# joesound212985/Deepfake-Detection-using-CLIP-Based-SigLIP-2-Vision-Transformers

Measured on AMD Instinct MI355X. Metric: images/sec (train fwd+bwd) SigLIP-2-so400m@384 bf16, higher is better.
Workload: dtype bf16; 1 GPU; so400m-patch14-384 encoder+pool-head train fwd+bwd, 384x384, per-GPU batch 128, seeded random weights; global_batch=128, parallelism=dp1

## Files before the change

deepfake-detection-using-clip-based-siglip-2-vision-transformers_amd/csrc/attention.hip:

```cpp
#include <stdlib.h>

#include "common.hip.h"
#include "kernels.h"

namespace sgl {

hipError_t attn_f32_fwd(const float*, const float*, const float*, float*, float*, int, int, int, int, int, int, hipStream_t);
hipError_t attn_f32_bwd(const float*, const float*, const float*, const float*, const float*, const float*, float*,
                        float*, int, int, int, int, int, int, hipStream_t);
hipError_t attn_ref_fwd(const float*, const float*, const float*, float*, float*, int, int, int, int, int, int, hipStream_t);
hipError_t attn_ref_bwd(const float*, const float*, const float*, const float*, const float*, const float*, float*,
                        float*, int, int, int, int, int, int, hipStream_t);

template <int DP>
struct AttnCfg {
  static constexpr int KS = DP / 16;
  static constexpr int DT = (DP + 31) / 32;
  static constexpr int CPR = DP / 8;
  static constexpr int RSTR = DP * 2 + 16;
  static constexpr int TSTR = 192;
  static constexpr int DSTR = 208;
};

__device__ __forceinline__ u32x4 a_ldg(__amdgpu_buffer_rsrc_t r, uint32_t off) {
  return __builtin_amdgcn_raw_buffer_load_b128(r, off, 0, 0);
}
template <typename T>
__device__ __forceinline__ lo_x8<T> as_x8(u32x4 v) { return __builtin_bit_cast(lo_x8<T>, v); }
template <typename T>
__device__ __forceinline__ lo_x8<T> lds_row8(const char* p) { return *reinterpret_cast<const lo_x8<T>*>(p); }
template <typename T>
__device__ __forceinline__ lo_x4<T> lds_tr4(const char* p) { return lds_read_tr16<T>(p); }
template <typename T>
__device__ __forceinline__ lo_x8<T> lds_trfrag(const char* img, int stride, int kk, int dcol0, int lane) {
  const int g = lane >> 4, q = (lane >> 2) & 3, p = lane & 3;
  const char* a = img + (16 * kk + 4 * (g >> 1) + q) * stride + (dcol0 + 16 * (g & 1) + 4 * p) * 2;
  const lo_x4<T> lo = lds_tr4<T>(a);
  const lo_x4<T> hi = lds_tr4<T>(a + 8 * stride);
  return __builtin_shufflevector(lo, hi, 0, 1, 2, 3, 4, 5, 6, 7);
}
template <typename T>
__device__ __forceinline__ lo_x8<T> pack8(const f32x16& s, int base) {
  lo_x8<T> r;
#pragma unroll
  for (int j = 0; j < 8; ++j) r[j] = (T)s[base + j];
  return r;
}
__device__ __forceinline__ float fast_exp2(float x) { return __builtin_amdgcn_exp2f(x); }

__device__ __forceinline__ bool head_block(int nb, int BH, int& bh, int& xb) {
  const int pid = blockIdx.x, xcd = pid & 7, slot = pid >> 3;
  const int hq = slot / nb;
  bh = hq * 8 + xcd;
  xb = slot - hq * nb;
  return bh < BH;
}
static inline dim3 head_grid(int nb, int BH) { return dim3((unsigned)(8 * ((BH + 7) / 8) * nb)); }

struct HeadSrc {
  uint32_t rowbytes, nc, bytes;
  size_t base;
};
__device__ __forceinline__ HeadSrc head_src(int ld, int b, int hd, int H, int N, int dh, int DP) {
  HeadSrc r;
  if (ld > 0) {
    r.rowbytes = (uint32_t)ld * 2u;
    r.nc = (uint32_t)dh / 8u;
    r.bytes = (uint32_t)(((size_t)(N - 1) * ld + dh) * 2);
    r.base = (size_t)b * N * ld + (size_t)hd * dh;
  } else {
    r.rowbytes = (uint32_t)DP * 2u;
    r.nc = (uint32_t)DP / 8u;
    r.bytes = (uint32_t)((size_t)N * DP * 2);
    r.base = ((size_t)b * H + hd) * (size_t)N * DP;
  }
  return r;
}

#define MFMA32(a, b, c) mfma_32x32x16((a), (b), (c))

__device__ __forceinline__ void att_dma16(u32x4 desc, uint32_t lds_addr, uint32_t voff) {
  asm volatile("s_mov_b32 m0, %0\n\ts_nop 0\n\tbuffer_load_dwordx4 %1, %2, 0 offen lds" ::"s"(lds_addr), "v"(voff), "s"(desc)
               : "memory");
}
__device__ __forceinline__ void att_dma4(u32x4 desc, uint32_t lds_addr, uint32_t voff) {
  asm volatile("s_mov_b32 m0, %0\n\ts_nop 0\n\tbuffer_load_dword %1, %2, 0 offen lds" ::"s"(lds_addr), "v"(voff), "s"(desc)
               : "memory");
}
__device__ __forceinline__ u32x4 att_desc(const void* base, uint32_t bytes) {
  const uint64_t q = (uint64_t)base;
  return u32x4{(uint32_t)q, (uint32_t)(q >> 32) & 0xffffu, bytes, 0x00020000u};
}
__device__ __forceinline__ uint32_t att_chunk_off(int cidx, int rows, int SC, int NC, uint32_t rowbytes) {
  const int row = cidx / SC, col = cidx - row * SC;
  return (row < rows && col < NC) ? (uint32_t)row * rowbytes + (uint32_t)col * 16u : SGL_OOB;
}
#define SGL_ATT_WAIT_BARRIER(n)                                   \
  do {                                                            \
    asm volatile("s_waitcnt vmcnt(" #n ") lgkmcnt(0)" ::: "memory"); \
    __builtin_amdgcn_sched_barrier(0);                            \
    __builtin_amdgcn_s_barrier();                                 \
    __builtin_amdgcn_sched_barrier(0);                            \
    asm volatile("" ::: "memory");                                \
  } while (0)

template <typename T, int DP, bool TOK>
__global__ __launch_bounds__(256) __attribute__((amdgpu_waves_per_eu(3, 3))) void attn_fwd_kernel(const T* __restrict__ Q, const T* __restrict__ K,
                                                          const T* __restrict__ V, T* __restrict__ out,
                                                          float* __restrict__ lse, int B, int H, int N, int dh, int ld,
                                                          float c, float scale) {
  using C = AttnCfg<DP>;
  constexpr int KT = 64;
  constexpr int KBYTES = KT * C::RSTR, VBYTES = KT * C::TSTR, STAGE = KBYTES + VBYTES;
  constexpr int SCK = C::RSTR / 16, SCV = C::TSTR / 16;
  constexpr int NIK = KT * SCK / 64, NIV = KT * SCV / 64, NSLOT = NIK + NIV;
  constexpr int NPW = (NSLOT + 3) / 4;
  static_assert(KT * SCK % 64 == 0 && KT * SCV % 64 == 0, "whole DMA instructions per image");
  extern __shared__ __attribute__((aligned(16))) char smem[];
  const int t = threadIdx.x, lane = t & 63;
  const int w = __builtin_amdgcn_readfirstlane(t >> 6);
  int bh, xb;
  if (!head_block((N + 127) / 128, B * H, bh, xb)) return;
  const int b = bh / H, hd = bh - b * H;
  const int q0 = xb * 128 + w * 32;
  HeadSrc src = head_src(TOK ? ld : 0, b, hd, H, N, dh, DP);
  if constexpr (!TOK) {
    src.rowbytes = (uint32_t)DP * 2u;
    src.nc = (uint32_t)DP / 8u;
  }
  const __amdgpu_buffer_rsrc_t rq = make_rsrc(Q + src.base, src.bytes);
  const u32x4 dk_ = att_desc(K + src.base, src.bytes);
  const u32x4 dv_ = att_desc(V + src.base, src.bytes);
  const uint32_t lds0 = (uint32_t)(size_t)((SGL_LDS char*)smem);

  const int qi = lane & 31, hh = lane >> 5;
  lo_x8<T> qf[C::KS];
#pragma unroll
  for (int ks = 0; ks < C::KS; ++ks) {
    const uint32_t ch = (uint32_t)(2 * ks + hh);
    qf[ks] = as_x8<T>(a_ldg(rq, (q0 + qi < N && ch < src.nc) ? (uint32_t)(q0 + qi) * src.rowbytes + ch * 16u : SGL_OOB));
  }

  uint32_t voff[NPW];
#pragma unroll
  for (int j = 0; j < NPW; ++j) {
    const int sl = w + 4 * j;
    voff[j] = (sl < NIK) ? att_chunk_off(sl * 64 + lane, KT, SCK, (int)src.nc, src.rowbytes)
                         : att_chunk_off((sl - NIK) * 64 + lane, KT, SCV, (int)src.nc, src.rowbytes);
  }
  const uint32_t tile_adv = (uint32_t)KT * src.rowbytes;
  auto issue = [&](int stage) {
    const uint32_t sb = lds0 + (uint32_t)(stage * STAGE);
#pragma unroll
    for (int j = 0; j < NPW; ++j) {
      const int sl = w + 4 * j;
      if (sl < NSLOT) att_dma16(sl < NIK ? dk_ : dv_, sb + (uint32_t)sl * 1024u, voff[j]);
      voff[j] += tile_adv;
    }
  };

  float m_run = -INFINITY, l_run = 0.f;
  f32x16 o[C::DT];
#pragma unroll
  for (int dt = 0; dt < C::DT; ++dt)
#pragma unroll
    for (int r = 0; r < 16; ++r) o[dt][r] = 0.f;

  const int ntiles = (N + KT - 1) / KT;
#pragma unroll
  for (int ks = 0; ks < C::KS; ++ks) asm volatile("" ::"v"(qf[ks]));
  asm volatile("s_waitcnt vmcnt(0)" ::: "memory");
  issue(0);
  for (int tile = 0; tile < ntiles; ++tile) {
    const int cur = tile & 1;
    SGL_ATT_WAIT_BARRIER(0);
    if (tile + 1 < ntiles) issue(cur ^ 1);
    const char* kb = smem + cur * STAGE;
    const char* vb = kb + KBYTES;
    f32x16 s0, s1;
#pragma unroll
    for (int r = 0; r < 16; ++r) { s0[r] = 0.f; s1[r] = 0.f; }
#pragma unroll
    for (int ks = 0; ks < C::KS; ++ks) {
      const lo_x8<T> k0 = lds_row8<T>(kb + qi * C::RSTR + (16 * ks + 8 * hh) * 2);
      const lo_x8<T> k1 = lds_row8<T>(kb + (qi + 32) * C::RSTR + (16 * ks + 8 * hh) * 2);
      s0 = MFMA32(k0, qf[ks], s0);
      s1 = MFMA32(k1, qf[ks], s1);
    }
    if (tile == ntiles - 1) {
#pragma unroll
      for (int r = 0; r < 16; ++r) {
        const int key = tile * KT + (r & 3) + 8 * (r >> 2) + 4 * hh;
        if (key >= N) s0[r] = -INFINITY;
        if (key + 32 >= N) s1[r] = -INFINITY;
      }
    }
    float mx = s0[0];
#pragma unroll
    for (int r = 1; r < 16; ++r) mx = fmaxf(mx, s0[r]);
#pragma unroll
    for (int r = 0; r < 16; ++r) mx = fmaxf(mx, s1[r]);
    mx = fmaxf(mx, __shfl_xor(mx, 32, 64));
    const float m_new = fmaxf(m_run, mx);
    const bool grew = __any(m_new > m_run);
    const float alpha = grew ? fast_exp2(c * (m_run - m_new)) : 1.0f;
    const float mc = m_new * c;
    float rs = 0.f;
#pragma unroll
    for (int r = 0; r < 16; ++r) {
      s0[r] = fast_exp2(fmaf(s0[r], c, -mc));
      s1[r] = fast_exp2(fmaf(s1[r], c, -mc));
      rs += s0[r] + s1[r];
    }
    l_run = l_run * alpha + rs;
    m_run = m_new;
    if (grew) {
#pragma unroll
      for (int dt = 0; dt < C::DT; ++dt)
#pragma unroll
        for (int r = 0; r < 16; ++r) o[dt][r] *= alpha;
    }
    lo_x8<T> pb[4];
    pb[0] = pack8<T>(s0, 0);
    pb[1] = pack8<T>(s0, 8);
    pb[2] = pack8<T>(s1, 0);
    pb[3] = pack8<T>(s1, 8);
#pragma unroll
    for (int dt = 0; dt < C::DT; ++dt)
#pragma unroll
      for (int kk = 0; kk < 4; ++kk) o[dt] = MFMA32(lds_trfrag<T>(vb, C::TSTR, kk, dt * 32, lane), pb[kk], o[dt]);
  }
  const float l = l_run + __shfl_xor(l_run, 32, 64);
  const float inv = 1.0f / l;
  const int q = q0 + qi;
  if (q < N) {
    T* orow = out + ((size_t)b * N + q) * ((size_t)H * dh) + hd * dh;
#pragma unroll
    for (int dt = 0; dt < C::DT; ++dt)
#pragma unroll
      for (int g4 = 0; g4 < 4; ++g4) {
        const int d = dt * 32 + 8 * g4 + 4 * hh;
        if (d < dh) {
          lo_x4<T> v4;
#pragma unroll
          for (int r = 0; r < 4; ++r) v4[r] = (T)(o[dt][4 * g4 + r] * inv);
          *reinterpret_cast<lo_x4<T>*>(orow + d) = v4;
        }
      }
    if (hh == 0) lse[(size_t)bh * N + q] = m_run * scale + __logf(l);
  }
}

template <typename T, int DP, bool TOK>
__global__ __launch_bounds__(256, 2) void attn_bwd_kv_kernel(const T* __restrict__ Q, const T* __restrict__ K,
                                                             const T* __restrict__ V, const T* __restrict__ dO,
                                                             const float* __restrict__ aux, T* __restrict__ dqkv,
                                                             int B, int H, int N, int dh, int ld, float c, float scale) {
  using C = AttnCfg<DP>;
  constexpr int QT = 32;
  constexpr int SC = C::DSTR / 16;
  constexpr int NIS = (QT * SC + 63) / 64;
  constexpr int IMG = NIS * 1024;
  constexpr int STAGE = 2 * IMG + QT * 8;
  constexpr int NSLOT = 2 * NIS + 1;
  static_assert(NSLOT <= 16 && NSLOT > 12, "four DMA slots per wave (three for the last wave)");
  extern __shared__ __attribute__((aligned(16))) char smem[];
  const int t = threadIdx.x, lane = t & 63;
  const int w = __builtin_amdgcn_readfirstlane(t >> 6);
  int bh, xb;
  if (!head_block((N + 127) / 128, B * H, bh, xb)) return;
  const int b = bh / H, hd = bh - b * H;
  const int D = H * dh;
  const int key0 = xb * 128 + w * 32;
  HeadSrc src = head_src(TOK ? ld : 0, b, hd, H, N, dh, DP);
  if constexpr (!TOK) {
    src.rowbytes = (uint32_t)DP * 2u;
    src.nc = (uint32_t)DP / 8u;
  }
  const __amdgpu_buffer_rsrc_t rk = make_rsrc(K + src.base, src.bytes);
  const __amdgpu_buffer_rsrc_t rv = make_rsrc(V + src.base, src.bytes);
  const T* dOb = dO + (size_t)b * N * D + hd * dh;
  const u32x4 dq_ = att_desc(Q + src.base, src.bytes);
  const u32x4 ddo = att_desc(dOb, (uint32_t)(((size_t)(N - 1) * D + dh) * 2));
  const u32x4 dax = att_desc(aux + (size_t)bh * N * 2, (uint32_t)((size_t)N * 8));
  const uint32_t lds0 = (uint32_t)(size_t)((SGL_LDS char*)smem);

  const int li = lane & 31, hh = lane >> 5;
  lo_x8<T> kfr[C::KS], vfr[C::KS];
#pragma unroll
  for (int ks = 0; ks < C::KS; ++ks) {
    const uint32_t ch = (uint32_t)(2 * ks + hh);
    const uint32_t off = (key0 + li < N && ch < src.nc) ? (uint32_t)(key0 + li) * src.rowbytes + ch * 16u : SGL_OOB;
    kfr[ks] = as_x8<T>(a_ldg(rk, off));
    vfr[ks] = as_x8<T>(a_ldg(rv, off));
  }

  uint32_t voff[4], vadv[4];
  u32x4 dsc[3];
#pragma unroll
  for (int j = 0; j < 4; ++j) {
    const int sl = w + 4 * j;
    if (sl < NIS) {
      voff[j] = att_chunk_off(sl * 64 + lane, QT, SC, (int)src.nc, src.rowbytes);
      vadv[j] = (uint32_t)QT * src.rowbytes;
    } else if (sl < 2 * NIS) {
      voff[j] = att_chunk_off((sl - NIS) * 64 + lane, QT, SC, dh / 8, (uint32_t)D * 2u);
      vadv[j] = (uint32_t)(QT * D * 2);
    } else {
      voff[j] = (uint32_t)lane * 4u;
      vadv[j] = (uint32_t)(QT * 8);
    }
    if (j < 3) dsc[j] = (sl < NIS) ? dq_ : ddo;
  }
  auto issue1 = [&](int j, int stage) {
    const uint32_t sb = lds0 + (uint32_t)(stage * STAGE) + (uint32_t)w * 1024u;
    if (j < 3) {
      att_dma16(dsc[j], sb + (uint32_t)j * 4096u, voff[j]);
    } else {
      if (w < 2) att_dma16(ddo, sb + 3u * 4096u, voff[3]);
      else if (w == 2) att_dma4(dax, lds0 + (uint32_t)(stage * STAGE + 2 * IMG), voff[3]);
    }
    voff[j] += vadv[j];
  };
  auto issue = [&](int stage) {
#pragma unroll
    for (int j = 0; j < 4; ++j) issue1(j, stage);
  };

  f32x16 dk[C::DT], dv[C::DT];
#pragma unroll
  for (int dt = 0; dt < C::DT; ++dt)
#pragma unroll
    for (int r = 0; r < 16; ++r) { dk[dt][r] = 0.f; dv[dt][r] = 0.f; }

  const int ntiles = (N + QT - 1) / QT;
#pragma unroll
  for (int ks = 0; ks < C::KS; ++ks) asm volatile("" ::"v"(kfr[ks]), "v"(vfr[ks]));
  asm volatile("s_waitcnt vmcnt(0)" ::: "memory");
  issue(0);
  issue(1);
  int st = 0;
  for (int qt = 0; qt < ntiles; ++qt) {
    if (w == 3) SGL_ATT_WAIT_BARRIER(3); else SGL_ATT_WAIT_BARRIER(4);
    const int st_next = (st == 0) ? 2 : st - 1;
    const char* qimg = smem + st * STAGE;
    const char* dimg = qimg + IMG;
    const float* ld = reinterpret_cast<const float*>(qimg + 2 * IMG);
    st = (st == 2) ? 0 : st + 1;
    f32x16 S, dP;
#pragma unroll
    for (int r = 0; r < 16; ++r) { S[r] = 0.f; dP[r] = 0.f; }
    lo_x8<T> qa[C::KS], da[C::KS];
#pragma unroll
    for (int ks = 0; ks < C::KS; ++ks) {
      qa[ks] = lds_row8<T>(qimg + li * C::DSTR + (16 * ks + 8 * hh) * 2);
      da[ks] = lds_row8<T>(dimg + li * C::DSTR + (16 * ks + 8 * hh) * 2);
    }
#pragma unroll
    for (int ks = 0; ks < C::KS; ++ks) {
      S = MFMA32(qa[ks], kfr[ks], S);
      dP = MFMA32(da[ks], vfr[ks], dP);
    }
    if constexpr (C::KS == 5) {
      __builtin_amdgcn_sched_group_barrier(0x100, 4, 0);
#pragma unroll
      for (int i = 0; i < 6; ++i) {
        __builtin_amdgcn_sched_group_barrier(0x008, 1, 0);
        __builtin_amdgcn_sched_group_barrier(0x100, 1, 0);
      }
      __builtin_amdgcn_sched_group_barrier(0x008, 4, 0);
    }
    __builtin_amdgcn_sched_barrier(0);
    constexpr int NF = 2 * 2 * C::DT;
    lo_x8<T> fr[NF];
    auto frag = [&](int i) {
      const int which = i & 1, kk = (i >> 1) & 1, dt = i >> 2;
      return lds_trfrag<T>(which ? qimg : dimg, C::DSTR, kk, dt * 32, lane);
    };
    constexpr int PRE = NF < 2 ? NF : 2;
#pragma unroll
    for (int i = 0; i < PRE; ++i) fr[i] = frag(i);
    __builtin_amdgcn_sched_barrier(0);
#pragma unroll
    for (int g4 = 0; g4 < 4; ++g4) {
      const f32x4 A0 = *reinterpret_cast<const f32x4*>(ld + 2 * (8 * g4 + 4 * hh));
      const f32x4 A1 = *reinterpret_cast<const f32x4*>(ld + 2 * (8 * g4 + 4 * hh) + 4);
      const float L4[4] = {A0[0], A0[2], A1[0], A1[2]};
      const float D4[4] = {A0[1], A0[3], A1[1], A1[3]};
#pragma unroll
      for (int r3 = 0; r3 < 4; ++r3) {
        const int r = 4 * g4 + r3;
        const float p = fast_exp2(fmaf(S[r], c, L4[r3]));
        S[r] = p;
        dP[r] = p * fmaf(dP[r], scale, D4[r3]);
      }
    }
    lo_x8<T> pb[2], dsb[2];
    pb[0] = pack8<T>(S, 0);
    pb[1] = pack8<T>(S, 8);
    dsb[0] = pack8<T>(dP, 0);
    dsb[1] = pack8<T>(dP, 8);
    __builtin_amdgcn_sched_barrier(0);
#pragma unroll
    for (int i = 0; i < NF; ++i) {
      if (i + PRE < NF) fr[i + PRE] = frag(i + PRE);
      const int which = i & 1, kk = (i >> 1) & 1, dt = i >> 2;
      if (which) dk[dt] = MFMA32(fr[i], dsb[kk], dk[dt]);
      else dv[dt] = MFMA32(fr[i], pb[kk], dv[dt]);
      if (i % 3 == 1) issue1(i / 3, st_next);
      __builtin_amdgcn_sched_barrier(0);
    }
#pragma unroll
    for (int j = (NF + 1) / 3; j < 4; ++j) issue1(j, st_next);
  }
  asm volatile("s_waitcnt vmcnt(0)" ::: "memory");
  const int key = key0 + li;
  if (key < N) {
    T* krow = dqkv + ((size_t)b * N + key) * (3 * (size_t)D) + D + hd * dh;
    T* vrow = krow + D;
#pragma unroll
    for (int dt = 0; dt < C::DT; ++dt)
#pragma unroll
      for (int g4 = 0; g4 < 4; ++g4) {
        const int d = dt * 32 + 8 * g4 + 4 * hh;
        if (d < dh) {
          lo_x4<T> a, g;
#pragma unroll
          for (int r = 0; r < 4; ++r) {
            a[r] = (T)dk[dt][4 * g4 + r];
            g[r] = (T)dv[dt][4 * g4 + r];
          }
          *reinterpret_cast<lo_x4<T>*>(krow + d) = a;
          *reinterpret_cast<lo_x4<T>*>(vrow + d) = g;
        }
      }
  }
}

template <typename T, int DP, bool TOK>
__global__ __launch_bounds__(256, 2) void attn_bwd_q_kernel(const T* __restrict__ Q, const T* __restrict__ K,
                                                            const T* __restrict__ V, const T* __restrict__ O,
                                                            const T* __restrict__ dO, const float* __restrict__ lse,
                                                            float* __restrict__ aux, T* __restrict__ dqkv,
                                                            int B, int H, int N, int dh, int ld, float c, float scale) {
  using C = AttnCfg<DP>;
  constexpr int KT = 32;
  constexpr int SCK = C::DSTR / 16, SCV = C::RSTR / 16;
  constexpr int NIK = (KT * SCK + 63) / 64, NIV = (KT * SCV + 63) / 64;
  constexpr int KIMG = NIK * 1024, VIMG = NIV * 1024, STAGE = KIMG + VIMG;
  constexpr int NSLOT = NIK + NIV;
  static_assert(NSLOT <= 16, "at most four DMA slots per wave");
  constexpr float LOG2E = 1.4426950408889634f;
  extern __shared__ __attribute__((aligned(16))) char smem[];
  const int t = threadIdx.x, lane = t & 63;
  const int w = __builtin_amdgcn_readfirstlane(t >> 6);
  int bh, xb;
  if (!head_block((N + 127) / 128, B * H, bh, xb)) return;
  const int b = bh / H, hd = bh - b * H;
  const int D = H * dh;
  const int q0 = xb * 128 + w * 32;
  HeadSrc src = head_src(TOK ? ld : 0, b, hd, H, N, dh, DP);
  if constexpr (!TOK) {
    src.rowbytes = (uint32_t)DP * 2u;
    src.nc = (uint32_t)DP / 8u;
  }
  const __amdgpu_buffer_rsrc_t rq = make_rsrc(Q + src.base, src.bytes);
  const T* dOb = dO + (size_t)b * N * D + hd * dh;
  const __amdgpu_buffer_rsrc_t rdo = make_rsrc(dOb, (uint32_t)(((size_t)(N - 1) * D + dh) * 2));
  const u32x4 dk_ = att_desc(K + src.base, src.bytes);
  const u32x4 dv_ = att_desc(V + src.base, src.bytes);
  const uint32_t lds0 = (uint32_t)(size_t)((SGL_LDS char*)smem);

  const int li = lane & 31, hh = lane >> 5;
  const int q = q0 + li;
  lo_x8<T> qf[C::KS], dof[C::KS];
#pragma unroll
  for (int ks = 0; ks < C::KS; ++ks) {
    const int col = 16 * ks + 8 * hh;
    qf[ks] = as_x8<T>(a_ldg(rq, (q < N && (uint32_t)(col >> 3) < src.nc) ? (uint32_t)q * src.rowbytes + (uint32_t)col * 2u
                                                                           : SGL_OOB));
    dof[ks] = as_x8<T>(a_ldg(rdo, (q < N && col < dh) ? (uint32_t)(((size_t)q * D + col) * 2) : SGL_OOB));
  }
  float dl = 0.f;
  {
    const __amdgpu_buffer_rsrc_t ro = make_rsrc(O + (size_t)b * N * D + hd * dh, (uint32_t)(((size_t)(N - 1) * D + dh) * 2));
#pragma unroll
    for (int ks = 0; ks < C::KS; ++ks) {
      const int col = 16 * ks + 8 * hh;
      const lo_x8<T> of = as_x8<T>(a_ldg(ro, (q < N && col < dh) ? (uint32_t)(((size_t)q * D + col) * 2) : SGL_OOB));
#pragma unroll
      for (int j = 0; j < 8; ++j) dl = fmaf((float)of[j], (float)dof[ks][j], dl);
    }
    dl += __shfl_xor(dl, 32, 64);
  }
  const float Lq = (q < N) ? -lse[(size_t)bh * N + q] * LOG2E : -INFINITY;
  const float Dq = (q < N) ? -dl * scale : 0.f;
  if (q < N && hh == 0) *reinterpret_cast<float2*>(aux + 2 * ((size_t)bh * N + q)) = make_float2(Lq, Dq);

  uint32_t voff[4];
  u32x4 dsc[4];
  uint32_t ldst[4];
#pragma unroll
  for (int j = 0; j < 4; ++j) {
    const int sl = w + 4 * j;
    if (sl < NIK) {
      voff[j] = att_chunk_off(sl * 64 + lane, KT, SCK, (int)src.nc, src.rowbytes);
      dsc[j] = dk_;
      ldst[j] = (uint32_t)sl * 1024u;
    } else {
      voff[j] = att_chunk_off((sl - NIK) * 64 + lane, KT, SCV, (int)src.nc, src.rowbytes);
      dsc[j] = dv_;
      ldst[j] = (uint32_t)(KIMG + (sl - NIK) * 1024);
    }
  }
  auto issue1 = [&](int j, int stage) {
    if (w + 4 * j < NSLOT) att_dma16(dsc[j], lds0 + (uint32_t)(stage * STAGE) + ldst[j], voff[j]);
    voff[j] += (uint32_t)KT * src.rowbytes;
  };

  f32x16 dq[C::DT];
#pragma unroll
  for (int dt = 0; dt < C::DT; ++dt)
#pragma unroll
    for (int r = 0; r < 16; ++r) dq[dt][r] = 0.f;

  const int ntiles = (N + KT - 1) / KT;
#pragma unroll
  for (int ks = 0; ks < C::KS; ++ks) asm volatile("" ::"v"(qf[ks]), "v"(dof[ks]));
  asm volatile("" ::"v"(Lq), "v"(Dq));
  asm volatile("s_waitcnt vmcnt(0)" ::: "memory");
#pragma unroll
  for (int j = 0; j < 4; ++j) issue1(j, 0);
#pragma unroll
  for (int j = 0; j < 4; ++j) issue1(j, 1);
  int st = 0;
  for (int kt = 0; kt < ntiles; ++kt) {
    const int nw = (NSLOT - w + 3) / 4;
    if (nw >= 4) SGL_ATT_WAIT_BARRIER(4);
    else if (nw == 3) SGL_ATT_WAIT_BARRIER(3);
    else if (nw == 2) SGL_ATT_WAIT_BARRIER(2);
    else SGL_ATT_WAIT_BARRIER(1);
    const int st_next = (st == 0) ? 2 : st - 1;
    const char* kimg = smem + st * STAGE;
    const char* vimg = kimg + KIMG;
    st = (st == 2) ? 0 : st + 1;
    f32x16 S, dP;
#pragma unroll
    for (int r = 0; r < 16; ++r) { S[r] = 0.f; dP[r] = 0.f; }
    lo_x8<T> ka[C::KS], va[C::KS];
#pragma unroll
    for (int ks = 0; ks < C::KS; ++ks) {
      ka[ks] = lds_row8<T>(kimg + li * C::DSTR + (16 * ks + 8 * hh) * 2);
      va[ks] = lds_row8<T>(vimg + li * C::RSTR + (16 * ks + 8 * hh) * 2);
    }
#pragma unroll
    for (int ks = 0; ks < C::KS; ++ks) {
      S = MFMA32(ka[ks], qf[ks], S);
      dP = MFMA32(va[ks], dof[ks], dP);
    }
    if constexpr (C::KS == 5) {
      __builtin_amdgcn_sched_group_barrier(0x100, 6, 0);
#pragma unroll
      for (int i = 0; i < 4; ++i) {
        __builtin_amdgcn_sched_group_barrier(0x008, 1, 0);
        __builtin_amdgcn_sched_group_barrier(0x100, 1, 0);
      }
      __builtin_amdgcn_sched_group_barrier(0x008, 6, 0);
    }
    __builtin_amdgcn_sched_barrier(0);
    lo_x8<T> kt_frag[C::DT][2];
#pragma unroll
    for (int dt = 0; dt < C::DT; ++dt)
#pragma unroll
      for (int kk = 0; kk < 2; ++kk) kt_frag[dt][kk] = lds_trfrag<T>(kimg, C::DSTR, kk, dt * 32, lane);
    __builtin_amdgcn_sched_barrier(0);
#pragma unroll
    for (int r = 0; r < 16; ++r) {
      const float p = fast_exp2(fmaf(S[r], c, Lq));
      dP[r] = p * fmaf(dP[r], scale, Dq);
    }
    if (kt == ntiles - 1) {
#pragma unroll
      for (int r = 0; r < 16; ++r) {
        const int key = kt * KT + (r & 3) + 8 * (r >> 2) + 4 * hh;
        if (key >= N) dP[r] = 0.f;
      }
    }
    lo_x8<T> dsb[2];
    dsb[0] = pack8<T>(dP, 0);
    dsb[1] = pack8<T>(dP, 8);
#pragma unroll
    for (int i = 0; i < 2 * C::DT; ++i) {
      dq[i >> 1] = MFMA32(kt_frag[i >> 1][i & 1], dsb[i & 1], dq[i >> 1]);
      if (i < 4) issue1(i, st_next);
      __builtin_amdgcn_sched_barrier(0);
    }
#pragma unroll
    for (int j = 2 * C::DT; j < 4; ++j) issue1(j, st_next);
  }
  asm volatile("s_waitcnt vmcnt(0)" ::: "memory");
  if (q < N) {
    T* qrow = dqkv + ((size_t)b * N + q) * (3 * (size_t)D) + hd * dh;
#pragma unroll
    for (int dt = 0; dt < C::DT; ++dt)
#pragma unroll
      for (int g4 = 0; g4 < 4; ++g4) {
        const int d = dt * 32 + 8 * g4 + 4 * hh;
        if (d < dh) {
          lo_x4<T> a;
#pragma unroll
          for (int r = 0; r < 4; ++r) a[r] = (T)dq[dt][4 * g4 + r];
          *reinterpret_cast<lo_x4<T>*>(qrow + d) = a;
        }
      }
  }
}

template <typename T, int DP>
static hipError_t fwd_launch(const T* q, const T* k, const T* v, T* out, float* lse, int B, int H, int N,
                             int dh, int ld, hipStream_t s) {
  using C = AttnCfg<DP>;
  constexpr int smem = 2 * (64 * C::RSTR + 64 * C::TSTR);
  const float scale = 1.0f / sqrtf((float)dh);
  if (ld > 0)
    hipLaunchKernelGGL((attn_fwd_kernel<T, DP, true>), head_grid((N + 127) / 128, B * H), dim3(256), smem, s, q, k, v, out, lse,
                       B, H, N, dh, ld, scale * 1.4426950408889634f, scale);
  else
    hipLaunchKernelGGL((attn_fwd_kernel<T, DP, false>), head_grid((N + 127) / 128, B * H), dim3(256), smem, s, q, k, v, out,
                       lse, B, H, N, dh, 0, scale * 1.4426950408889634f, scale);
  return hipGetLastError();
}

template <typename T, int DP>
static hipError_t bwd_launch(const T* q, const T* k, const T* v, const T* out, const T* dout,
                             const float* lse, T* dqkv, float* delta, int B, int H, int N, int dh, int ld,
                             hipStream_t s) {
  using C = AttnCfg<DP>;
  const float scale = 1.0f / sqrtf((float)dh);
  const float c = scale * 1.4426950408889634f;
  constexpr int smem_kv = 3 * (2 * ((32 * (C::DSTR / 16) + 63) / 64) * 1024 + 32 * 8);
  constexpr int smem_q = 3 * (((32 * (C::DSTR / 16) + 63) / 64) + ((32 * (C::RSTR / 16) + 63) / 64)) * 1024;
  const dim3 grid = head_grid((N + 127) / 128, B * H), block(256);
  if (ld > 0)
    hipLaunchKernelGGL((attn_bwd_q_kernel<T, DP, true>), grid, block, smem_q, s, q, k, v, out, dout, lse, delta, dqkv, B, H, N,
                       dh, ld, c, scale);
  else
    hipLaunchKernelGGL((attn_bwd_q_kernel<T, DP, false>), grid, block, smem_q, s, q, k, v, out, dout, lse, delta, dqkv, B, H, N,
                       dh, 0, c, scale);
  hipError_t e = hipGetLastError();
  if (e != hipSuccess) return e;
  if (ld > 0)
    hipLaunchKernelGGL((attn_bwd_kv_kernel<T, DP, true>), grid, block, smem_kv, s, q, k, v, dout, delta, dqkv, B, H, N, dh, ld, c,
                       scale);
  else
    hipLaunchKernelGGL((attn_bwd_kv_kernel<T, DP, false>), grid, block, smem_kv, s, q, k, v, dout, delta, dqkv, B, H, N, dh, 0,
                       c, scale);
  return hipGetLastError();
}

static bool attn_shape_ok(int N, int dh, int DP, int H, int ld) {
  if (dh % 8 || DP != ((dh + 15) / 16) * 16) return false;
  if (DP != 16 && DP != 32 && DP != 48 && DP != 64 && DP != 80 && DP != 96) return false;
  if (ld < 0 || (ld > 0 && (ld % 8 || ld < H * dh))) return false;
  if ((size_t)N * (ld > 0 ? ld : DP) * 2 >= (1ull << 31)) return false;
  if ((size_t)N * H * dh * 2 >= (1ull << 31)) return false;
  return true;
}

hipError_t attn_fwd(const void* q, const void* k, const void* v, int dtype, void* out, float* lse, int B, int H, int N,
                    int dh, int DP, int ld, hipStream_t s) {
  if (B * H == 0 || N == 0) return hipSuccess;
  if (dtype == DT_F32)
    return attn_ref_fwd((const float*)q, (const float*)k, (const float*)v, (float*)out, lse, B, H, N, dh, DP, ld, s);
  if (dtype == DT_F32_MFMA)
    return attn_f32_fwd((const float*)q, (const float*)k, (const float*)v, (float*)out, lse, B, H, N, dh, DP, ld, s);
  if (!attn_shape_ok(N, dh, DP, H, ld)) return hipErrorInvalidValue;
  if ((((uintptr_t)q) | ((uintptr_t)k) | ((uintptr_t)v)) & 15) return hipErrorInvalidValue;
#define SGL_F(T, DPV) \
  case DPV: return fwd_launch<T, DPV>((const T*)q, (const T*)k, (const T*)v, (T*)out, lse, B, H, N, dh, ld, s);
  if (dtype == DT_F16) {
    switch (DP) {
      SGL_F(f16, 16) SGL_F(f16, 32) SGL_F(f16, 48) SGL_F(f16, 64) SGL_F(f16, 80) SGL_F(f16, 96)
    }
    return hipErrorInvalidValue;
  }
  switch (DP) {
    SGL_F(bf16, 16) SGL_F(bf16, 32) SGL_F(bf16, 48) SGL_F(bf16, 64) SGL_F(bf16, 80) SGL_F(bf16, 96)
  }
#undef SGL_F
  return hipErrorInvalidValue;
}

hipError_t attn_bwd(const void* q, const void* k, const void* v, const void* out, const void* dout, const float* lse,
                    int dtype, void* dqkv, float* delta, float* , int B, int H, int N, int dh, int DP,
                    int ld, hipStream_t s) {
  if (B * H == 0 || N == 0) return hipSuccess;
  if (dtype == DT_F32)
    return attn_ref_bwd((const float*)q, (const float*)k, (const float*)v, (const float*)out, (const float*)dout, lse,
                        (float*)dqkv, delta, B, H, N, dh, DP, ld, s);
  if (dtype == DT_F32_MFMA)
    return attn_f32_bwd((const float*)q, (const float*)k, (const float*)v, (const float*)out, (const float*)dout, lse,
                        (float*)dqkv, delta, B, H, N, dh, DP, ld, s);
  if (!attn_shape_ok(N, dh, DP, H, ld)) return hipErrorInvalidValue;
  if ((((uintptr_t)q) | ((uintptr_t)k) | ((uintptr_t)v)) & 15) return hipErrorInvalidValue;
#define SGL_B(T, DPV)                                                                                  \
  case DPV:                                                                                            \
    return bwd_launch<T, DPV>((const T*)q, (const T*)k, (const T*)v, (const T*)out, (const T*)dout, lse, \
                              (T*)dqkv, delta, B, H, N, dh, ld, s);
  if (dtype == DT_F16) {
    switch (DP) {
      SGL_B(f16, 16) SGL_B(f16, 32) SGL_B(f16, 48) SGL_B(f16, 64) SGL_B(f16, 80) SGL_B(f16, 96)
    }
    return hipErrorInvalidValue;
  }
  switch (DP) {
    SGL_B(bf16, 16) SGL_B(bf16, 32) SGL_B(bf16, 48) SGL_B(bf16, 64) SGL_B(bf16, 80) SGL_B(bf16, 96)
  }
#undef SGL_B
  return hipErrorInvalidValue;
}

}
```

Baseline: 441.1 images/sec.

## Interleave K/V DMA issues and LDS fragment prefetch with MFMAs in attention forward

Replaces the bulk issue of the next tile's K/V DMA at the top of each iteration with one DMA slot issued after each MFMA. K and V LDS fragments are software-prefetched a few MFMAs ahead, and sched_barriers pin the order. The softmax exp and bf16 packing are split into halves, and the alpha rescale uses inline-asm v_mul so the compiler cannot fuse or reorder it. The aim is to hide LDS and global-load latency behind matrix math, at the cost of extra register pressure and a rigid schedule that may stall if the compiler would have done better.

```diff
diff --git a/deepfake-detection-using-clip-based-siglip-2-vision-transformers_amd/csrc/attention.hip b/deepfake-detection-using-clip-based-siglip-2-vision-transformers_amd/csrc/attention.hip
--- a/deepfake-detection-using-clip-based-siglip-2-vision-transformers_amd/csrc/attention.hip
+++ b/deepfake-detection-using-clip-based-siglip-2-vision-transformers_amd/csrc/attention.hip
@@ -47,6 +47,11 @@
   return r;
 }
 __device__ __forceinline__ float fast_exp2(float x) { return __builtin_amdgcn_exp2f(x); }
+__device__ __forceinline__ float mul1_f32(float a, float b) {
+  float r;
+  asm("v_mul_f32 %0, %1, %2" : "=v"(r) : "v"(a), "v"(b));
+  return r;
+}
 
 __device__ __forceinline__ bool head_block(int nb, int BH, int& bh, int& xb) {
   const int pid = blockIdx.x, xcd = pid & 7, slot = pid >> 3;
@@ -149,15 +154,19 @@
                          : att_chunk_off((sl - NIK) * 64 + lane, KT, SCV, (int)src.nc, src.rowbytes);
   }
   const uint32_t tile_adv = (uint32_t)KT * src.rowbytes;
-  auto issue = [&](int stage) {
-    const uint32_t sb = lds0 + (uint32_t)(stage * STAGE);
-#pragma unroll
-    for (int j = 0; j < NPW; ++j) {
-      const int sl = w + 4 * j;
-      if (sl < NSLOT) att_dma16(sl < NIK ? dk_ : dv_, sb + (uint32_t)sl * 1024u, voff[j]);
-      voff[j] += tile_adv;
-    }
+  auto issue1 = [&](int j, int stage) {
+    const int sl = w + 4 * j;
+    const uint32_t dst = lds0 + (uint32_t)(stage * STAGE) + (uint32_t)sl * 1024u;
+    if (4 * j + 3 < NSLOT || sl < NSLOT) {
+      if (4 * j + 3 < NIK) att_dma16(dk_, dst, voff[j]);
+      else if (4 * j >= NIK) att_dma16(dv_, dst, voff[j]);
+      else att_dma16(sl < NIK ? dk_ : dv_, dst, voff[j]);
+    }
+    voff[j] += tile_adv;
   };
+  constexpr int NFK = 2 * C::KS, PREK = NFK < 4 ? NFK : 4;
+  constexpr int NFV = 4 * C::DT, PREV = 4;
+  static_assert(NPW <= NFK + NFV - 1, "a DMA slot behind each of MFMAs 1 .. NPW");
 
   float m_run = -INFINITY, l_run = 0.f;
   f32x16 o[C::DT];
@@ -170,23 +179,37 @@
 #pragma unroll
   for (int ks = 0; ks < C::KS; ++ks) asm volatile("" ::"v"(qf[ks]));
   asm volatile("s_waitcnt vmcnt(0)" ::: "memory");
-  issue(0);
+#pragma unroll
+  for (int j = 0; j < NPW; ++j) issue1(j, 0);
   for (int tile = 0; tile < ntiles; ++tile) {
     const int cur = tile & 1;
     SGL_ATT_WAIT_BARRIER(0);
-    if (tile + 1 < ntiles) issue(cur ^ 1);
     const char* kb = smem + cur * STAGE;
     const char* vb = kb + KBYTES;
+    auto dma_behind = [&](int g) {
+      if (g >= 1 && g <= NPW) issue1(g - 1, cur ^ 1);
+    };
     f32x16 s0, s1;
 #pragma unroll
     for (int r = 0; r < 16; ++r) { s0[r] = 0.f; s1[r] = 0.f; }
-#pragma unroll
-    for (int ks = 0; ks < C::KS; ++ks) {
-      const lo_x8<T> k0 = lds_row8<T>(kb + qi * C::RSTR + (16 * ks + 8 * hh) * 2);
-      const lo_x8<T> k1 = lds_row8<T>(kb + (qi + 32) * C::RSTR + (16 * ks + 8 * hh) * 2);
-      s0 = MFMA32(k0, qf[ks], s0);
-      s1 = MFMA32(k1, qf[ks], s1);
-    }
+    lo_x8<T> kf[NFK];
+    auto kfrag = [&](int i) { return lds_row8<T>(kb + (qi + 32 * (i & 1)) * C::RSTR + (16 * (i >> 1) + 8 * hh) * 2); };
+#pragma unroll
+    for (int i = 0; i < PREK; ++i) kf[i] = kfrag(i);
+    __builtin_amdgcn_sched_barrier(0);
+#pragma unroll
+    for (int i = 0; i < NFK; ++i) {
+      if (i + PREK < NFK) kf[i + PREK] = kfrag(i + PREK);
+      if (i & 1) s1 = MFMA32(kf[i], qf[i >> 1], s1);
+      else s0 = MFMA32(kf[i], qf[i >> 1], s0);
+      dma_behind(i);
+      __builtin_amdgcn_sched_barrier(0);
+    }
+    lo_x8<T> fr[NFV];
+    auto vfrag = [&](int i) { return lds_trfrag<T>(vb, C::TSTR, i & 3, (i >> 2) * 32, lane); };
+#pragma unroll
+    for (int i = 0; i < PREV; ++i) fr[i] = vfrag(i);
+    __builtin_amdgcn_sched_barrier(0);
     if (tile == ntiles - 1) {
 #pragma unroll
       for (int r = 0; r < 16; ++r) {
@@ -206,30 +229,38 @@
     const float alpha = grew ? fast_exp2(c * (m_run - m_new)) : 1.0f;
     const float mc = m_new * c;
     float rs = 0.f;
-#pragma unroll
-    for (int r = 0; r < 16; ++r) {
-      s0[r] = fast_exp2(fmaf(s0[r], c, -mc));
-      s1[r] = fast_exp2(fmaf(s1[r], c, -mc));
-      rs += s0[r] + s1[r];
+    lo_x8<T> pb[4];
+#pragma unroll
+    for (int h = 0; h < 2; ++h) {
+#pragma unroll
+      for (int r = 8 * h; r < 8 * h + 8; ++r) {
+        s0[r] = fast_exp2(fmaf(s0[r], c, -mc));
+        s1[r] = fast_exp2(fmaf(s1[r], c, -mc));
+        rs += s0[r] + s1[r];
+      }
+      pb[h] = pack8<T>(s0, 8 * h);
+      pb[2 + h] = pack8<T>(s1, 8 * h);
+      if (h == 0) __builtin_amdgcn_sched_barrier(0);
     }
     l_run = l_run * alpha + rs;
+    asm volatile("" : "+v"(l_run));
     m_run = m_new;
     if (grew) {
 #pragma unroll
       for (int dt = 0; dt < C::DT; ++dt)
 #pragma unroll
-        for (int r = 0; r < 16; ++r) o[dt][r] *= alpha;
-    }
-    lo_x8<T> pb[4];
-    pb[0] = pack8<T>(s0, 0);
-    pb[1] = pack8<T>(s0, 8);
-    pb[2] = pack8<T>(s1, 0);
-    pb[3] = pack8<T>(s1, 8);
-#pragma unroll
-    for (int dt = 0; dt < C::DT; ++dt)
-#pragma unroll
-      for (int kk = 0; kk < 4; ++kk) o[dt] = MFMA32(lds_trfrag<T>(vb, C::TSTR, kk, dt * 32, lane), pb[kk], o[dt]);
-  }
+        for (int r = 0; r < 16; ++r) o[dt][r] = mul1_f32(o[dt][r], alpha);
+    }
+    __builtin_amdgcn_sched_barrier(0);
+#pragma unroll
+    for (int i = 0; i < NFV; ++i) {
+      if (i + PREV < NFV) fr[i + PREV] = vfrag(i + PREV);
+      o[i >> 2] = MFMA32(fr[i], pb[i & 3], o[i >> 2]);
+      dma_behind(NFK + i);
+      __builtin_amdgcn_sched_barrier(0);
+    }
+  }
+  asm volatile("s_waitcnt vmcnt(0)" ::: "memory");
   const float l = l_run + __shfl_xor(l_run, 32, 64);
   const float inv = 1.0f / l;
   const int q = q0 + qi;
```

After: 443.2 images/sec, median of 6. About the same (+0.5%).
